# Pose-Group/FAMI-Pose

Measured on AMD Instinct MI355X. Metric: train clips/sec (5-frame 384x288 HRNet-W48), higher is better.
Workload: dtype f32

## Files before the change

fami-pose_amd/csrc/conv.hip:

```cpp
#include "common.h"
#include <type_traits>
#include <string.h>

#include "conv_epi.h"
extern "C" int fami_conv2d_fwd_bnin_ok(int N, int H, int W, int Ci, int Co);
#include "conv_pair.h"
int fami_pair_launch(const PairCapture& c, hipStream_t s);


struct ConvArgs {
  EpiBN e;
  int emode;
  const float* x;
  const float* wp;
  float* y;
  const float* bias;
  const float* addend;
  int N, Hi, Wi, Ci, Ho, Wo, Co;
  int kh, kw, sh, pad, dil;
  int KC, NTt, relu, accumulate, P;
  unsigned x_bytes, wp_bytes;
  int xcd;
  int prio;
  int par;
// ... 2384 lines not shown
      static bool attr2 = false;                                                                                   \
      if (!attr2) {                                                                                                \
        (void)hipFuncSetAttribute((const void*)conv3x3_lds_kernel<T, nt, ksc, 1>, hipFuncAttributeMaxDynamicSharedMemorySize, 156 * 1024); \
        attr2 = true;                                                                                              \
      }                                                                                                            \
      hipLaunchKernelGGL((conv3x3_lds_kernel<T, nt, ksc, 1>), grid, dim3(256), lds, s, a);                         \
    } else                                                                                                         \
    hipLaunchKernelGGL((conv3x3_lds_kernel<T, nt, ksc>), grid, dim3(256), lds, s, a);                              \
    launched = true;                                                                                               \
  }
  FAMI_LDS_CASE(3, 1) FAMI_LDS_CASE(3, 2) FAMI_LDS_CASE(3, 3) FAMI_LDS_CASE(3, 4)
  FAMI_LDS_CASE(4, 1) FAMI_LDS_CASE(4, 2) FAMI_LDS_CASE(4, 3) FAMI_LDS_CASE(4, 4)
#undef FAMI_LDS_CASE
  if (!launched) return 0;
  hipError_t e = hipGetLastError();
  if (e != hipSuccess) {
    fami_set_error(name, hipGetErrorString(e));
    return FAMI_EHIP;
  }
  return 1;
}

static bool wgrad_lin_ok(int H, int W, int Ci, int Co, int kh, int kw, int stride, int pad, int dil) {
  return stride == 1 && 2 * pad == dil * (kh - 1) && 2 * pad == dil * (kw - 1) && kh * kw > 1 && kh * kw <= 9 && W >= 4 &&
         Ci % 16 == 0 && Co % 16 == 0;
}
static bool geom_ok(int kh, int kw, int stride, int pad, int dil) {
  return kh >= 1 && kw >= 1 && kh <= 7 && kw <= 7 && (stride == 1 || stride == 2) && pad >= 0 && dil >= 1;
}
static inline int out_dim(int i, int k, int stride, int pad, int dil) {
  return (i + 2 * pad - dil * (k - 1) - 1) / stride + 1;
}

extern "C" {
int fami_dcn_tune(int mode);
int fami_bn_tune_small(long elems);

int fami_conv_tune(int mt, int nt, int ks) {
  g_force_mt = mt; g_force_nt = nt; g_force_ks = ks;
  return FAMI_OK;
}
void fami_conv_stem_tune(int on);
int fami_conv_tune_lds(int on) {
  if (on == 9000 || on == 9001) {
    fami_conv_stem_tune(on - 9000);
    return FAMI_OK;
  }
  if (on < 0) fami_conv_stem_tune(-1);
  if (on == 10 || on == 11 || on == 20 || on == 21 || on == 30 || on == 31 || (on >= 40 && on <= 42) || (on >= 52 && on <= 54) || (on >= 60 && on <= 62) || on >= 100) {
    fami_conv_t4_tune(on);
    return FAMI_OK;
  }
  g_use_lds = on < 0 ? -1 : (on ? 1 : 0);
  g_lds_sim = on == 2;
  if (on < 0) fami_conv_t4_tune(-1);
  return FAMI_OK;
}
int fami_conv_tune_wgrad_lds(int on) {
  if (on >= 30000) {
    fami_wgrad_s3_tune(on - 30000);
    return FAMI_OK;
  }
  if (on >= 20000) {
    fami_wgrad16_tune(on - 20000);
    return FAMI_OK;
  }
  if (on >= 1000) {
    g_wgrad_ps = on - 1000;
    return FAMI_OK;
  }
  if (on >= 50 && on <= 54) {
    g_wgrad_lin = on - 50;
    return FAMI_OK;
  }
  if (on >= 100) {
    g_wgrad_mt = on - 100;
    return FAMI_OK;
  }
  if (on < 0) {
    fami_wgrad16_tune(-1);
    fami_wgrad_s3_tune(-1);
    g_wgrad_lds = 1;
    g_wgrad_lds_f32 = 2;
    g_wgrad_nsub = 2;
    g_wgrad_lin = 1;
    return FAMI_OK;
  }
  g_wgrad_lds = on ? 1 : 0;
  g_wgrad_lds_f32 = on ? 1 : 0;
  if (on > 1) g_wgrad_nsub = on - 1;
  return FAMI_OK;
}
int fami_conv_tune_xcd(int mode) {
  g_xcd = mode < 0 ? -1 : (mode & 1);
  g_xcd_w = mode < 0 ? 1 : ((mode >> 1) & 1);
  return FAMI_OK;
}
int fami_conv_tune_stages(int stages) {
  if (stages == 120 || stages == 121) {
    g_prio = stages - 120;
    return FAMI_OK;
  }
  if (stages == 110 || stages == 111) {
    g_par = stages - 110;
    return FAMI_OK;
  }
  if (stages == 100 || stages == 101) {
    g_lin_conv = stages - 100;
    return FAMI_OK;
  }
  g_stages = (stages >= 2 && stages <= 4) ? stages : 0;
  return FAMI_OK;
}
int fami_tune_reset(void) {
  fami_conv_tune(0, 0, 0);
  fami_conv_tune_lds(-1);
  fami_conv_tune_wgrad_lds(-1);
  fami_conv_tune_xcd(-1);
  g_stages = 0; g_prio = 0; g_lin_conv = 1; g_par = 1;
  g_wgrad_ps = 0; g_wgrad_mt = 0;
  fami_dcn_tune(-1);
  fami_bn_tune_small(-1);
  return FAMI_OK;
}
int fami_tune_defaults(int f32_split) {
  if (f32_split >= 0) {
    fami_conv_t4_default_split(f32_split);
    fami_wgrad_s3_default(f32_split);
  }
  return fami_tune_reset();
}

long fami_packed_weight_elems(int Co, int Ci, int kh, int kw, int mode) {
  const int kd = mode == 0 ? Ci : Co, nd = mode == 0 ? Co : Ci;
  return pack16_elems(kd, nd, kh * kw) + pack32_elems(kd, nd, kh * kw) + fami_split_image_elems(kd, nd, kh * kw);
}

int fami_pack_conv_weight_f32(const float* w_oihw, float* wp, int Co, int Ci, int kh, int kw, int mode,
                              hipStream_t s) {
  FAMI_REQUIRE(w_oihw && wp && Co > 0 && Ci > 0 && (mode == 0 || mode == 1), "fami_pack_conv_weight_f32", "bad argument");
  const int kd = mode == 0 ? Ci : Co, nd = mode == 0 ? Co : Ci;
  const long total = pack16_elems(kd, nd, kh * kw) + pack32_elems(kd, nd, kh * kw);
  hipLaunchKernelGGL(pack_w_kernel, dim3(fami_ew_grid(total)), dim3(256), 0, s, w_oihw, wp, Co, Ci, kh * kw, mode);
  FAMI_CHECK_LAUNCH("fami_pack_conv_weight_f32");
  if (fami_split_image_elems(kd, nd, kh * kw) > 0) {
    fami_pack_split_single(w_oihw, wp + total, Co, Ci, kh * kw, mode, s);
    FAMI_CHECK_LAUNCH("fami_pack_conv_weight_f32/split");
  }
  return FAMI_OK;
}

static int conv_fwd_f32_impl(const char* nm, const float* x, const float* wp, const float* bias, const float* addend,
                             float* y, int N, int H, int W, int Ci, int Co, int kh, int kw, int stride, int pad, int dil,
                             int relu, int accumulate, const EpiBN& e, hipStream_t s, const XBN& xbn = xbn_none());
int fami_conv2d_fwd_f32(const float* x, const float* wp, const float* bias, const float* addend, float* y, int N,
                        int H, int W, int Ci, int Co, int kh, int kw, int stride, int pad, int dil, int relu,
                        int accumulate, hipStream_t s) {
  return conv_fwd_f32_impl("fami_conv2d_fwd_f32", x, wp, bias, addend, y, N, H, W, Ci, Co, kh, kw, stride, pad, dil, relu,
                           accumulate, epi_none(), s);
}
int fami_conv2d_fwd_stats_f32(const float* x, const float* wp, const float* bias, float* y, int N, int H, int W, int Ci,
                              int Co, int kh, int kw, int stride, int pad, int dil, void* slots, const float* pivot_src,
                              hipStream_t s) {
  FAMI_REQUIRE(slots, "fami_conv2d_fwd_stats_f32", "null slots");
  EpiBN e = epi_none();
// ... 25 lines not shown
                             int relu, int accumulate, const EpiBN& e, hipStream_t s, const XBN& xbn) {
  FAMI_REQUIRE(x && wp && y && N > 0 && H > 0 && W > 0 && Ci > 0 && Co > 0, nm, "bad argument");
  if (!geom_ok(kh, kw, stride, pad, dil)) {
    fami_set_error(nm, "unsupported geometry");
    return FAMI_ESHAPE;
  }
  ConvArgs a;
  a.e = e; a.emode = e.slots ? e.mode : 0;
  a.x = x; a.wp = wp; a.y = y; a.bias = bias; a.addend = addend;
  a.N = N; a.Hi = H; a.Wi = W; a.Ci = Ci;
  a.Ho = out_dim(H, kh, stride, pad, dil); a.Wo = out_dim(W, kw, stride, pad, dil); a.Co = Co;
  a.kh = kh; a.kw = kw; a.sh = stride == 2 ? 1 : 0; a.pad = pad; a.dil = dil;
  a.KC = fami_cdiv(Ci, 16); a.NTt = fami_cdiv(Co, 16); a.relu = relu; a.accumulate = accumulate;
  const long P = (long)N * a.Ho * a.Wo;
  const long xb = (long)N * H * W * Ci * 4, wb = (long)kh * kw * a.KC * a.NTt * 1024;
  FAMI_REQUIRE(P > 0 && P < (1L << 31) && xb < (1L << 31) && wb < (1L << 31), nm, "tensor >= 2 GiB");
  a.P = (int)P; a.x_bytes = (unsigned)xb; a.wp_bytes = (unsigned)wb;
  if (Ci == 3 && !addend && !xbn.on) {
    const int rc = fami_try_conv_stem1(2, x, wp, bias, y, N, H, W, Ci, Co, kh, kw, stride, pad, dil, a.NTt, relu, accumulate, 1, s, nm, e);
    if (rc != 0) return rc < 0 ? rc : FAMI_OK;
  }
  if (kh == 3 && kw == 3 && stride == 1 && pad == 1 && dil == 1 && !addend) {
    const int rc = try_conv3x3_lds<float>(x, wp, bias, y, N, H, W, Ci, Co, a.KC, a.NTt, +1, relu, accumulate, 1, s, nm, e, xbn);
    if (rc != 0) return rc < 0 ? rc : FAMI_OK;
  }
  if (kh == 3 && kw == 3 && stride == 1 && pad == dil && dil > 1 && !addend && !e.slots && !xbn.on && g_use_lds != 0) {
    const int rc = fami_try_conv3x3_t4_dil(2, x, wp, bias, y, N, H, W, Ci, Co, a.KC, a.NTt, +1, relu, accumulate, 1, dil, s, nm);
    if (rc != 0) return rc < 0 ? rc : FAMI_OK;
  }
  if (xbn.on) {
    fami_set_error(nm, "input BatchNorm needs the split-product 3x3 kernel (ask fami_conv2d_xbn_ok_f32 first)");
    return FAMI_ESHAPE;
  }
  return run_igemm(a, 0, s, nm);
}
extern "C" {

static int conv_dgrad_f32_impl(const char* nm, const float* dy, const float* wp, const float* addend, float* dx, int N,
                               int H, int W, int Ci, int Co, int kh, int kw, int stride, int pad, int dil, int accumulate,
                               const EpiBN& e, hipStream_t s);
int fami_conv2d_dgrad_f32(const float* dy, const float* wp, const float* addend, float* dx, int N, int H, int W,
                          int Ci, int Co, int kh, int kw, int stride, int pad, int dil, int accumulate,
                          hipStream_t s) {
  return conv_dgrad_f32_impl("fami_conv2d_dgrad_f32", dy, wp, addend, dx, N, H, W, Ci, Co, kh, kw, stride, pad, dil,
                             accumulate, epi_none(), s);
}
int fami_conv2d_dgrad_bnstats_f32(const float* dy, const float* wp, float* dx, int N, int H, int W, int Ci, int Co,
                                  int kh, int kw, int stride, int pad, int dil, int accumulate, const float* z,
                                  const float* yrelu, const float* mean, const float* invstd, const float* gamma,
                                  const float* beta, int relu, void* slots, hipStream_t s) {
  FAMI_REQUIRE(slots && z && mean && invstd && gamma && beta && (relu != 1 || yrelu) && relu >= 0 && relu <= 2,
               "fami_conv2d_dgrad_bnstats_f32", "bad argument");
  EpiBN e = epi_none();
  e.slots = reinterpret_cast<double*>(slots); e.ns = bn_slots(Ci); e.mode = 2; e.relu = relu; e.C = Ci;
  e.z = z; e.yr = yrelu; e.mean = mean; e.invstd = invstd; e.gamma = gamma; e.beta = beta;
  return conv_dgrad_f32_impl("fami_conv2d_dgrad_bnstats_f32", dy, wp, nullptr, dx, N, H, W, Ci, Co, kh, kw, stride, pad,
                             dil, accumulate, e, s);
}
}
static int conv_dgrad_f32_impl(const char* nm, const float* dy, const float* wp, const float* addend, float* dx, int N,
                               int H, int W, int Ci, int Co, int kh, int kw, int stride, int pad, int dil, int accumulate,
                               const EpiBN& e, hipStream_t s) {
  FAMI_REQUIRE(dy && wp && dx && N > 0 && H > 0 && W > 0 && Ci > 0 && Co > 0, nm, "bad argument");
  if (!geom_ok(kh, kw, stride, pad, dil)) {
    fami_set_error(nm, "unsupported geometry");
    return FAMI_ESHAPE;
  }
  ConvArgs a;
  a.e = e; a.emode = e.slots ? e.mode : 0;
  a.x = dy; a.wp = wp; a.y = dx; a.bias = nullptr; a.addend = addend;
  a.N = N; a.Hi = out_dim(H, kh, stride, pad, dil); a.Wi = out_dim(W, kw, stride, pad, dil); a.Ci = Co;
  a.Ho = H; a.Wo = W; a.Co = Ci;
  a.kh = kh; a.kw = kw; a.sh = stride == 2 ? 1 : 0; a.pad = pad; a.dil = dil;
  a.KC = fami_cdiv(Co, 16); a.NTt = fami_cdiv(Ci, 16); a.relu = 0; a.accumulate = accumulate;
  const long P = (long)N * H * W;
  const long xb = (long)N * a.Hi * a.Wi * Co * 4, wb = (long)kh * kw * a.KC * a.NTt * 1024;
  FAMI_REQUIRE(P > 0 && P < (1L << 31) && xb < (1L << 31) && wb < (1L << 31), nm, "tensor >= 2 GiB");
  a.P = (int)P; a.x_bytes = (unsigned)xb; a.wp_bytes = (unsigned)wb;
  if (kh == 3 && kw == 3 && stride == 1 && pad == 1 && dil == 1 && !addend) {
    const int rc = try_conv3x3_lds<float>(dy, wp, nullptr, dx, N, H, W, Co, Ci, a.KC, a.NTt, -1, 0, accumulate, 1, s, nm, e);
    if (rc != 0) return rc < 0 ? rc : FAMI_OK;
  }
  if (kh == 3 && kw == 3 && stride == 1 && pad == dil && dil > 1 && !addend && !e.slots && g_use_lds != 0) {
    const int rc = fami_try_conv3x3_t4_dil(2, dy, wp, nullptr, dx, N, H, W, Co, Ci, a.KC, a.NTt, -1, 0, accumulate, 1, dil, s, nm);
    if (rc != 0) return rc < 0 ? rc : FAMI_OK;
  }
  return run_igemm(a, 1, s, nm);
}
extern "C" {

struct WgradPlan { int MT, NT, ciBlocks, coBlocks, psplit, chunk, pertap, w8; long P; };
static bool wgrad_lin_ok(int H, int W, int Ci, int Co, int kh, int kw, int stride, int pad, int dil);
static WgradPlan wgrad_plan(int N, int H, int W, int Ci, int Co, int kh, int kw, int stride, int pad, int dil, int w8 = 0) {
  WgradPlan q;
  const int Ho = out_dim(H, kh, stride, pad, dil), Wo = out_dim(W, kw, stride, pad, dil);
  q.P = (long)N * Ho * Wo;
  q.MT = pick_small(fami_cdiv(Ci, 16));
  q.NT = pick_small(fami_cdiv(Co, 16));
  if (g_wgrad_mt > 0 && g_wgrad_mt <= q.MT) q.MT = g_wgrad_mt;
  q.ciBlocks = fami_cdiv(fami_cdiv(Ci, 16), q.MT);
  q.coBlocks = fami_cdiv(fami_cdiv(Co, 16), q.NT);
  q.pertap = (kh * kw > 1 && kh * kw <= 9) ? 1 : 0;
  const long by = q.pertap ? (long)q.ciBlocks * q.coBlocks : (long)kh * kw * q.ciBlocks * q.coBlocks;
  long ps = ((q.pertap ? (g_wgrad_ps ? g_wgrad_ps : 512) : 1024) + by - 1) / by;
  q.w8 = 0;
  if (w8 == 3) w8 = 256 / by >= 16 ? 2 : 1;
  if (w8 && q.pertap && kh * kw == 9 && ps >= 9) {
    q.w8 = w8;
    const long T = (g_wgrad_ps ? g_wgrad_ps : (w8 == 2 ? 256 : 512)) / by;
    ps = T * 8 / 9;
    while (ps > 1 && ps + (ps + 7) / 8 > T) --ps;
    if (ps < 1) ps = 1;
    if (w8 == 2) ps *= 2;
  }
  const long maxps = q.pertap ? (q.P + 63) / 64 : (q.P + 255) / 256;
  if (ps > maxps) ps = maxps;
  if (ps < 1) ps = 1;
// ... 62 lines not shown
  G = (P + chunk - 1) / chunk;
  q.G = (int)G;
  q.chunk = (int)chunk;
  q.xbytes = (int)((chunk + 2 * (W + 1)) * q.xrow);
  q.lds = ((size_t)q.xbytes + (size_t)chunk * q.yrow + 16) * 4;
  q.ok = P < (1L << 31) && G < 65536;
  return q;
}

int fami_conv2d_xbn_ok(int N, int H, int W, int Ci, int Co) {
  return (g_use_lds != 0 && g_wgrad_lds && fami_conv_t4_eligible16(N, H, W, Ci, Co) &&
          fami_wgrad16_slabs(N, H, W, Ci, Co, 3, 1, 1, 1) > 0) ? 1 : 0;
}
long fami_conv2d_wgrad_workspace(int N, int H, int W, int Ci, int Co, int kh, int kw, int stride, int pad, int dil) {
  if (!geom_ok(kh, kw, stride, pad, dil)) return -1;
  const WgradPlan q = wgrad_plan(N, H, W, Ci, Co, kh, kw, stride, pad, dil);
  long need = (long)q.psplit * Co * Ci * kh * kw * (long)sizeof(float);
  const WgradLdsPlan l = wgrad_lds_plan(N, H, W, Ci, Co, kh, kw, stride, pad, dil);
  if (l.ok) {
    const long nl = (long)l.G * Co * Ci * 9 * (long)sizeof(float);
    if (nl > need) need = nl;
  }
  const WgradLdsPlan f = wgrad_lds_plan_f32(N, H, W, Ci, Co, kh, kw, stride, pad, dil);
  if (f.ok) {
    const long nl = (long)f.G * Co * Ci * 9 * (long)sizeof(float);
    if (nl > need) need = nl;
  }
  if (kh == kw) {
    const long nl = fami_wgrad16_slabs(N, H, W, Ci, Co, kh, stride, pad, dil) * Co * Ci * kh * kw * (long)sizeof(float);
    if (nl > need) need = nl;
  }
  if (kh == 3 && kw == 3 && stride == 1 && pad == 1 && dil == 1) {
    const long nl = fami_wgrad_s3_slabs(N, H, W, Ci, Co) * Co * Ci * 9 * (long)sizeof(float);
    if (nl > need) need = nl;
  }
  return need;
}

}

template <typename T>
static int wgrad_impl(const T* x, const T* dy, float* dw, float* workspace, long ws_bytes, int N, int H, int W, int Ci,
                      int Co, int kh, int kw, int stride, int pad, int dil, int accumulate, hipStream_t s,
                      const char* nm) {
  FAMI_REQUIRE(x && dy && dw && workspace && N > 0 && H > 0 && W > 0 && Ci > 0 && Co > 0, nm, "bad argument");
  if (!geom_ok(kh, kw, stride, pad, dil)) {
    fami_set_error(nm, "unsupported geometry");
    return FAMI_ESHAPE;
  }
  const bool lin = std::is_same<T, float>::value && g_wgrad_lin && wgrad_lin_ok(H, W, Ci, Co, kh, kw, stride, pad, dil);
  const WgradPlan q = wgrad_plan(N, H, W, Ci, Co, kh, kw, stride, pad, dil, !lin ? 0 : (g_wgrad_lin == 1 ? 3 : (g_wgrad_lin == 3 ? 1 : (g_wgrad_lin == 4 ? 2 : 0))));
  const long need = (long)q.psplit * Co * Ci * kh * kw * (long)sizeof(float);
  FAMI_REQUIRE(ws_bytes >= need, nm, "workspace too small");
  FAMI_REQUIRE(q.P < (1L << 31), nm, "size out of range");
  WgradArgs<T> a;
  a.x = x; a.dy = dy; a.part = workspace;
  a.N = N; a.H = H; a.W = W; a.Ci = Ci;
  a.Ho = out_dim(H, kh, stride, pad, dil); a.Wo = out_dim(W, kw, stride, pad, dil); a.Co = Co;
  a.kh = kh; a.kw = kw; a.sh = stride == 2 ? 1 : 0; a.pad = pad; a.dil = dil;
  a.P = (int)q.P; a.chunk = q.chunk; a.ciBlocks = q.ciBlocks; a.coBlocks = q.coBlocks; a.xcd = g_xcd_w; a.prio = g_prio;
  const long xb = (long)N * H * W * Ci * (long)sizeof(T), yb = q.P * Co * (long)sizeof(T);
  FAMI_REQUIRE(xb < (1L << 31) && yb < (1L << 31), nm, "tensor >= 2 GiB");
  a.x_bytes = (unsigned)xb; a.dy_bytes = (unsigned)yb;
  if (q.pertap) {
    const dim3 grid(q.w8 ? q.psplit + (q.psplit + 7) / 8 : q.psplit, q.ciBlocks * q.coBlocks), block(q.w8 ? 512 * q.w8 : kh * kw * 64);
    const size_t lin_lds = q.w8 == 2 ? (size_t)8 * q.MT * q.NT * 1024 : 0;
// ... 111 lines not shown
  if (rc != 0) {
    fami_set_error(name, "no kernel instance for tile shape");
    return FAMI_ESHAPE;
  }
  FAMI_CHECK_LAUNCH(name);
  return FAMI_OK;
}

extern "C" {

static int wgrad_f32_entry(const float* x, const float* dy, float* dw, float* workspace, long ws_bytes, int N, int H,
                           int W, int Ci, int Co, int kh, int kw, int stride, int pad, int dil, int accumulate,
                           hipStream_t s, const XBN& xbn);
int fami_conv2d_wgrad_f32(const float* x, const float* dy, float* dw, float* workspace, long ws_bytes, int N, int H,
                          int W, int Ci, int Co, int kh, int kw, int stride, int pad, int dil, int accumulate,
                          hipStream_t s) {
  return wgrad_f32_entry(x, dy, dw, workspace, ws_bytes, N, H, W, Ci, Co, kh, kw, stride, pad, dil, accumulate, s, xbn_none());
}
static int wgrad_f32_entry(const float* x, const float* dy, float* dw, float* workspace, long ws_bytes, int N, int H,
                           int W, int Ci, int Co, int kh, int kw, int stride, int pad, int dil, int accumulate,
                           hipStream_t s, const XBN& xbn) {
  if (kh == 3 && kw == 3 && stride == 1 && pad == 1 && dil == 1 && x && dy && dw && workspace) {
    const int G = fami_try_wgrad_s3(x, dy, workspace, ws_bytes, N, H, W, Ci, Co, s, "fami_conv2d_wgrad_f32", xbn);
    if (G < 0) return G;
    if (G > 0) {
      launch_reduce_taps(workspace, dw, Co, Ci, 9, G, accumulate, s);
      FAMI_CHECK_LAUNCH("fami_conv2d_wgrad_f32/reduce");
      return FAMI_OK;
    }
  }
  if (xbn.on) {
    fami_set_error("fami_conv2d_wgrad_defer_xbn_f32", "input BatchNorm needs the split-product kernel (ask fami_conv2d_xbn_ok_f32 first)");
    return FAMI_ESHAPE;
  }
  WgradLdsPlan l = g_wgrad_lds_f32 ? wgrad_lds_plan_f32(N, H, W, Ci, Co, kh, kw, stride, pad, dil) : WgradLdsPlan{0};
  if (g_wgrad_lds_f32 == 2 && l.ok &&
      (l.ciBlocks * l.coBlocks < 64 || (g_wgrad_lin && wgrad_lin_ok(H, W, Ci, Co, kh, kw, stride, pad, dil))))
    l.ok = 0;
  if (l.ok && x && dy && dw && workspace && ((reinterpret_cast<uintptr_t>(x) | reinterpret_cast<uintptr_t>(dy)) & 15) == 0) {
    const long need = (long)l.G * Co * Ci * 9 * (long)sizeof(float);
    FAMI_REQUIRE(ws_bytes >= need, "fami_conv2d_wgrad_f32", "workspace too small");
    WgradLdsArgsF a;
    a.x = x; a.dy = dy; a.part = workspace;
    a.N = N; a.H = H; a.W = W; a.Ci = Ci; a.Co = Co; a.P = N * H * W;
    a.chunk = l.chunk; a.ciBlocks = l.ciBlocks; a.coBlocks = l.coBlocks; a.xcd = g_xcd_w;
    a.CiB = 16 * l.CIT; a.CoB = 16 * l.COT; a.xrow = l.xrow; a.yrow = l.yrow; a.xfloats = l.xbytes;
    const dim3 grid(l.G, l.ciBlocks * l.coBlocks);
    bool ok = false;
#define FAMI_WF_CASE(cit, cot)                                                                                        \
  if (l.CIT == cit && l.COT == cot) {                                                                                 \
    static bool attr = false;                                                                                         \
    if (!attr) {                                                                                                      \
      (void)hipFuncSetAttribute((const void*)conv_wgrad_lds_f32_kernel<cit, cot>, hipFuncAttributeMaxDynamicSharedMemorySize, 160 * 1024); \
      attr = true;                                                                                                    \
    }                                                                                                                 \
    hipLaunchKernelGGL((conv_wgrad_lds_f32_kernel<cit, cot>), grid, dim3(512), l.lds, s, a);                          \
    ok = true;                                                                                                        \
  }
    FAMI_WF_CASE(1, 1) FAMI_WF_CASE(1, 2) FAMI_WF_CASE(1, 3) FAMI_WF_CASE(1, 4) FAMI_WF_CASE(2, 1) FAMI_WF_CASE(2, 2)
    FAMI_WF_CASE(2, 3) FAMI_WF_CASE(2, 4) FAMI_WF_CASE(3, 1) FAMI_WF_CASE(3, 2) FAMI_WF_CASE(3, 3) FAMI_WF_CASE(3, 4)
    FAMI_WF_CASE(4, 1) FAMI_WF_CASE(4, 2) FAMI_WF_CASE(4, 3) FAMI_WF_CASE(4, 4)
#undef FAMI_WF_CASE
    if (ok) {
      FAMI_CHECK_LAUNCH("fami_conv2d_wgrad_f32/lds");
      launch_reduce_taps(workspace, dw, Co, Ci, 9, l.G, accumulate, s);
      FAMI_CHECK_LAUNCH("fami_conv2d_wgrad_f32/reduce");
// ... 437 lines not shown
```

fami-pose_amd/csrc/conv_epi.h:

```cpp
#pragma once
#include "common.h"

struct EpiBN {
  double* slots;
  int ns, mode, relu, C;
  const float* pivot_src;
  const void* z;
  const void* yr;
  const float *mean, *invstd, *gamma, *beta;
};
static inline EpiBN epi_none() {
  EpiBN e;
  e.slots = nullptr; e.ns = 1; e.mode = 0; e.relu = 0; e.C = 0; e.pivot_src = nullptr; e.z = nullptr; e.yr = nullptr;
  e.mean = e.invstd = e.gamma = e.beta = nullptr;
  return e;
}
#if defined(__HIP_DEVICE_COMPILE__)
typedef const __attribute__((address_space(4))) EpiBN* EpiPtr;
__device__ __forceinline__ EpiPtr epi_late(unsigned off) {
  const __attribute__((address_space(4))) char* k =
      (const __attribute__((address_space(4))) char*)__builtin_amdgcn_kernarg_segment_ptr() + off;
  asm volatile("" : "+s"(k) : : "memory");
  return (EpiPtr)k;
}
// ... 61 lines not shown
}
template <typename H>
__device__ __forceinline__ u32x4 xbn_piece(u32x4 raw, const float* sc, const float* sf) {
  typedef H hx8 __attribute__((ext_vector_type(8)));
  typedef float f32x8 __attribute__((ext_vector_type(8)));
  f32x8 v = __builtin_convertvector(__builtin_bit_cast(hx8, raw), f32x8);
#pragma unroll
  for (int j = 0; j < 8; ++j) v[j] = fmaxf(__builtin_fmaf(v[j], sc[j], sf[j]), 0.f);
  return __builtin_bit_cast(u32x4, __builtin_convertvector(v, hx8));
}

int fami_try_conv3x3_t4(int half_kind, const void* x, const void* wp, const float* bias, void* y, int N, int H, int W, int Ci,
                        int Co, int KC, int NTt, int sgn, int relu, int accumulate, int out_f32, hipStream_t s,
                        const char* name, const EpiBN& epi, const XBN& xbn = xbn_none());
int fami_try_conv3x3_t4_dil(int half_kind, const void* x, const void* wp, const float* bias, void* y, int N, int H, int W, int Ci,
                            int Co, int KC, int NTt, int sgn, int relu, int accumulate, int out_f32, int dil, hipStream_t s,
                            const char* name);
void fami_conv_t4_tune(int on);
void fami_conv_t4_default_split(int on);
int fami_conv_t4_eligible16(int N, int H, int W, int Ci, int Co);
int fami_conv_t4_eligible_s3(int N, int H, int W, int Ci, int Co);

long fami_wgrad16_slabs(int N, int H, int W, int Ci, int Co, int k, int st, int pad, int dil);
int fami_try_wgrad16(int half_kind, const void* x, const void* dy, float* part, long ws_bytes, int N, int H, int W, int Ci,
                     int Co, int k, int st, int pad, int dil, hipStream_t s, const char* name, const XBN& xbn = xbn_none());
void fami_wgrad16_tune(int on);

long fami_wgrad_s3_slabs(int N, int H, int W, int Ci, int Co);
int fami_try_wgrad_s3(const float* x, const float* dy, float* part, long ws_bytes, int N, int H, int W, int Ci, int Co,
                      hipStream_t s, const char* name, const XBN& xbn = xbn_none());
void fami_wgrad_s3_tune(int on);
void fami_wgrad_s3_default(int on);

long fami_split_image_elems(int kd, int nd, int taps);
void fami_pack_split_single(const float* w_oihw, float* split, int Co, int Ci, int taps, int mode, hipStream_t s);
void fami_pack_split_batch(const float* params, float* packed, const void* desc, int n, hipStream_t s);
int fami_try_conv3x3_t5(int half_kind, const void* x, const void* wp, const float* bias, void* y, int N, int H, int W, int Ci,
                        int Co, int KC, int NTt, int sgn, int relu, int accumulate, int out_f32, hipStream_t s,
                        const char* name, const EpiBN& epi, const XBN& xbn);
void fami_conv_t5_tune(int on);
int fami_conv_t5_eligible_s3(int N, int H, int W, int Ci, int Co);

int fami_try_conv3x3_t6(int half_kind, const void* x, const void* wp, const float* bias, void* y, int N, int H, int W, int Ci,
                        int Co, int KC, int NTt, int sgn, int relu, int accumulate, int out_f32, hipStream_t s,
                        const char* name, const EpiBN& epi, const XBN& xbn);
extern "C" int fami_conv_t6_eligible(int N, int H, int W, int Ci, int Co);
void fami_conv_t6_tune(int on);
```

fami-pose_amd/csrc/route.h:

```cpp
#pragma once
#include "../../include/fami_route.h"
extern "C" fami_route_t* fami_rt(void);

#define g_dcn_gather (fami_rt()->dcn_gather)
#define g_dcn_abl (fami_rt()->dcn_abl)
#define g_dcn_win_r (fami_rt()->dcn_win_r)
#define g_dcn_ksplit (fami_rt()->dcn_ksplit)
#define g_dcn_pf (fami_rt()->dcn_pf)
#define g_dcn_bwd2 (fami_rt()->dcn_bwd2)
#define g_dcn_bwd2_cap (fami_rt()->dcn_bwd2_cap)
#define g_dcn_bwd2_stage (fami_rt()->dcn_bwd2_stage)
#define g_dcn_bwd_abl (fami_rt()->dcn_bwd_abl)
#define g_dcn_bwd_scatter (fami_rt()->dcn_bwd_scatter)
#define g_prio (fami_rt()->prio)
#define g_lin_conv (fami_rt()->lin_conv)
#define g_par (fami_rt()->par)
#define g_force_mt (fami_rt()->force_mt)
#define g_force_nt (fami_rt()->force_nt)
#define g_force_ks (fami_rt()->force_ks)
#define g_stages (fami_rt()->stages)
#define g_use32 (fami_rt()->use32)
#define g_xcd_w (fami_rt()->xcd_w)
#define g_xcd (fami_rt()->xcd)
#define g_use_lds (fami_rt()->use_lds)
// ... 26 lines not shown
#define g_t5_min_tiles (fami_rt()->t5_min_tiles)
#define g_use_t6 (fami_rt()->use_t6)
#define g_t6_rows (fami_rt()->t6_rows)
#define g_t6_min_jobs (fami_rt()->t6_min_jobs)
#define g_t6_mt (fami_rt()->t6_mt)
#define g_t7_target (fami_rt()->t7_target)
#define g_use_t7 (fami_rt()->use_t7)
#define g_t7_rows (fami_rt()->t7_rows)
#define g_t7_c64 (fami_rt()->t7_c64)
#define g_bn_in (fami_rt()->bn_in)
#define g_bwd_pair (fami_rt()->bwd_pair)
#define g_pair_wg6_target (fami_rt()->pair_wg6_target)
#define g_wg6_s2 (fami_rt()->wg6_s2)
#define g_wg6_dil (fami_rt()->wg6_dil)
#define g_wg6_c42 (fami_rt()->wg6_c42)
#define g_wg6_c4 (fami_rt()->wg6_c4)
#define g_wg6 (fami_rt()->wg6)
#define g_wg6_nu (fami_rt()->wg6_nu)
#define g_wg6_target (fami_rt()->wg6_target)
#define g_wg6_target_c4 (fami_rt()->wg6_target_c4)
#define g_wg1 (fami_rt()->wg1)
#define g_wg1_target (fami_rt()->wg1_target)
#define g_wgs (fami_rt()->wgs)
#define g_wg16_abl (fami_rt()->wg16_abl)
#define g_wg16 (fami_rt()->wg16)
#define g_wg16_bt (fami_rt()->wg16_bt)
#define g_wg16_target (fami_rt()->wg16_target)
#define g_wg16_general (fami_rt()->wg16_general)
#define g_wg16_bt18 (fami_rt()->wg16_bt18)
#define g_wgs3 (fami_rt()->wgs3)
#define g_wgs3_bt (fami_rt()->wgs3_bt)
#define g_wgs3_target (fami_rt()->wgs3_target)
#define g_wgs3_default (fami_rt()->wgs3_default)
#define g_bn_small_elems (fami_rt()->bn_small_elems)
#define g_bn2_maxg (fami_rt()->bn2_maxg)

static inline void fami_route_set_defaults(fami_route_t* q) {
  q->size = (int)sizeof(fami_route_t);
  q->dcn_gather = -1;
  q->dcn_abl = 0;
  q->dcn_win_r = 0;
  q->dcn_ksplit = 1;
  q->dcn_pf = 0;
  q->dcn_bwd2 = 1;
  q->dcn_bwd2_cap = 36;
  q->dcn_bwd2_stage = 1;
  q->dcn_bwd_abl = 0;
  q->dcn_bwd_scatter = -1;
  q->prio = 0;
  q->lin_conv = 1;
  q->par = 1;
  q->force_mt = 0;
  q->force_nt = 0;
  q->force_ks = 0;
  q->stages = 0;
  q->use32 = 1;
  q->xcd_w = 1;
  q->xcd = -1;
  q->use_lds = -1;
  q->lds_sim = 0;
  q->wgrad_nsub = 2;
  q->wgrad_ps = 0;
  q->wgrad_mt = 0;
  q->wgrad_lds = 1;
  q->wgrad_lds_f32 = 2;
  q->wgrad_lin = 1;
// ... 19 lines not shown
  q->t5_min_tiles = 0;
  q->use_t6 = 1;
  q->t6_rows = 0;
  q->t6_min_jobs = 96;
  q->t6_mt = 0;
  q->t7_target = 240;
  q->use_t7 = 1;
  q->t7_rows = 0;
  q->t7_c64 = 1;
  q->bn_in = 1;
  q->bwd_pair = 1;
  q->pair_wg6_target = 64;
  q->wg6_s2 = 1;
  q->wg6_dil = 1;
  q->wg6_c42 = 1;
  q->wg6_c4 = 1;
  q->wg6 = 1;
  q->wg6_nu = 0;
  q->wg6_target = 80;
  q->wg6_target_c4 = 160;
  q->wg1 = 1;
  q->wg1_target = 192;
  q->wgs = 1;
  q->wg16_abl = 0;
  q->wg16 = 1;
  q->wg16_bt = 0;
  q->wg16_target = 0;
  q->wg16_general = 1;
  q->wg16_bt18 = 0;
  q->wgs3 = 1;
  q->wgs3_bt = 0;
  q->wgs3_target = 0;
  q->wgs3_default = 1;
  q->bn_small_elems = 32768;
  q->bn2_maxg = 512;
}
```

include/fami.h:

```cpp
#ifndef FAMI_H
#define FAMI_H
#ifdef __cplusplus
extern "C" {
#endif

typedef void* fami_stream_t;

#include "fami_route.h"
long fami_route_size(void);
int fami_route_init(fami_route_t* route);
int fami_route_bind(fami_route_t* route);

const char* fami_version(void);
const char* fami_last_error(void);
int fami_device_info(int device, int* info, char* name, int name_len);

int fami_conv_tune(int mt, int nt, int ks);
int fami_conv_tune_lds(int on);
int fami_conv_tune_wgrad_lds(int on);
int fami_conv_tune_xcd(int mode);
int fami_conv_tune_stages(int stages);
int fami_tune_reset(void);
int fami_tune_defaults(int f32_split);
int fami_conv_t5_eligible(int N, int H, int W, int Ci, int Co);
int fami_conv_t6_eligible(int N, int H, int W, int Ci, int Co);
long fami_packed_weight_elems(int Co, int Ci, int kh, int kw, int mode);
int fami_pack_conv_weight_f32(const float* w_oihw, float* wp, int Co, int Ci, int kh, int kw, int mode,
                              fami_stream_t stream);
int fami_pack_conv_weights_batch_f32(const float* params, float* packed, const void* desc, int n, fami_stream_t stream);
int fami_conv2d_fwd_f32(const float* x, const float* wp, const float* bias, const float* addend, float* y, int N,
                        int H, int W, int Ci, int Co, int kh, int kw, int stride, int pad, int dil, int relu,
                        int accumulate, fami_stream_t stream);
int fami_conv2d_dgrad_f32(const float* dy, const float* wp, const float* addend, float* dx, int N, int H, int W,
                          int Ci, int Co, int kh, int kw, int stride, int pad, int dil, int accumulate,
                          fami_stream_t stream);
int fami_conv2d_fwd_stats_f32(const float* x, const float* wp, const float* bias, float* y, int N, int H, int W, int Ci,
                              int Co, int kh, int kw, int stride, int pad, int dil, void* slots, const float* pivot_src,
                              fami_stream_t stream);
int fami_conv2d_dgrad_bnstats_f32(const float* dy, const float* wp, float* dx, int N, int H, int W, int Ci, int Co,
                                  int kh, int kw, int stride, int pad, int dil, int accumulate, const float* z,
                                  const float* yrelu, const float* mean, const float* invstd, const float* gamma,
                                  const float* beta, int relu, void* slots, fami_stream_t stream);
long fami_conv2d_wgrad_workspace(int N, int H, int W, int Ci, int Co, int kh, int kw, int stride, int pad, int dil);
int fami_wgrad_reduce_desc_longs(void);
int fami_wgrad_reduce_batch(const long* descs, int n, fami_stream_t stream);
int fami_conv2d_wgrad_defer_f32(const float* x, const float* dy, float* dw, float* workspace, long ws_bytes, int N,
                                int H, int W, int Ci, int Co, int kh, int kw, int stride, int pad, int dil,
                                int accumulate, long* desc_out, fami_stream_t stream);
int fami_conv2d_wgrad_f32(const float* x, const float* dy, float* dw, float* workspace, long ws_bytes, int N, int H,
                          int W, int Ci, int Co, int kh, int kw, int stride, int pad, int dil, int accumulate,
                          fami_stream_t stream);

long fami_bn_workspace(int C);
int fami_bn_stats_f32(const float* x, long P, int C, float* mean, float* invstd, float* running_mean,
                      float* running_var, float momentum, float eps, float* ws, fami_stream_t stream);
int fami_bn_train_fwd_f32(const float* x, const float* residual, float* y, const float* gamma, const float* beta,
                          float* mean, float* invstd, float* running_mean, float* running_var, long P, int C,
                          int relu, float momentum, float eps, float* ws, fami_stream_t stream);
// ... 446 lines not shown
```

include/fami_route.h:

```cpp
#ifndef FAMI_ROUTE_H
#define FAMI_ROUTE_H
#ifdef __cplusplus
extern "C" {
#endif

typedef struct fami_route_t {
  int size;
  int  dcn_gather;
  int  dcn_abl;
  int  dcn_win_r;
  int  dcn_ksplit;
  int  dcn_pf;
  int  dcn_bwd2;
  int  dcn_bwd2_cap;
  int  dcn_bwd2_stage;
  int  dcn_bwd_abl;
  int  dcn_bwd_scatter;
  int  prio;
  int  lin_conv;
  int  par;
  int  force_mt;
  int  force_nt;
  int  force_ks;
  int  stages;
// ... 30 lines not shown
  int  t5_min_tiles;
  int  use_t6;
  int  t6_rows;
  int  t6_min_jobs;
  int  t6_mt;
  int  t7_target;
  int  use_t7;
  int  t7_rows;
  int  t7_c64;
  int  bn_in;
  int  bwd_pair;
  int  pair_wg6_target;
  int  wg6_s2;
  int  wg6_dil;
  int  wg6_c42;
  int  wg6_c4;
  int  wg6;
  int  wg6_nu;
  int  wg6_target;
  int  wg6_target_c4;
  int  wg1;
  int  wg1_target;
  int  wgs;
  int  wg16_abl;
  int  wg16;
  int  wg16_bt;
  int  wg16_target;
  int  wg16_general;
  int  wg16_bt18;
  int  wgs3;
  int  wgs3_bt;
  int  wgs3_target;
  int  wgs3_default;
  long bn_small_elems;
  int  bn2_maxg;
} fami_route_t;

#ifdef __cplusplus
}
#endif
#endif
```

Measured before the change: 90.98.

## Add streaming MFMA kernels for large 1x1 conv dgrad and wgrad

Adds a dedicated 1x1 convolution path: a persistent GEMM kernel with double-buffered LDS pixel tiles and MFMA 32x32x2 f32 for forward/dgrad (with optional BN-stats epilogue), and a wgrad kernel that streams pixel chunks into per-workgroup slabs reduced afterwards. By default it routes only large-P wgrad and Ci=64 dgrad shapes to the new kernels, replacing the generic implicit-GEMM path. This targets the generic path's overhead on skinny 1x1 GEMMs, at the cost of extra workspace for the slabs and more tuning knobs.

```diff
diff --git a/fami-pose_amd/csrc/conv.hip b/fami-pose_amd/csrc/conv.hip
--- a/fami-pose_amd/csrc/conv.hip
+++ b/fami-pose_amd/csrc/conv.hip
@@ -2440,6 +2440,11 @@
   return (i + 2 * pad - dil * (k - 1) - 1) / stride + 1;
 }
 
+static inline unsigned long c1s_addr_or(const void* a, const void* b, const void* c, const void* d, const void* e) {
+  return (unsigned long)(reinterpret_cast<uintptr_t>(a) | reinterpret_cast<uintptr_t>(b) | reinterpret_cast<uintptr_t>(c) |
+                         reinterpret_cast<uintptr_t>(d) | reinterpret_cast<uintptr_t>(e));
+}
+
 extern "C" {
 int fami_dcn_tune(int mode);
 int fami_bn_tune_small(long elems);
@@ -2505,6 +2510,14 @@
   return FAMI_OK;
 }
 int fami_conv_tune_stages(int stages) {
+  if (stages >= 130 && stages <= 132) {
+    g_c1s = stages - 130;
+    return FAMI_OK;
+  }
+  if (stages >= 1000) {
+    g_c1s_maxwg = stages - 1000;
+    return FAMI_OK;
+  }
   if (stages == 120 || stages == 121) {
     g_prio = stages - 120;
     return FAMI_OK;
@@ -2527,6 +2540,7 @@
   fami_conv_tune_xcd(-1);
   g_stages = 0; g_prio = 0; g_lin_conv = 1; g_par = 1;
   g_wgrad_ps = 0; g_wgrad_mt = 0;
+  g_c1s = 2; g_c1s_maxwg = 0;
   fami_dcn_tune(-1);
   fami_bn_tune_small(-1);
   return FAMI_OK;
@@ -2539,6 +2553,11 @@
   return fami_tune_reset();
 }
 
+int fami_conv1x1_stream_eligible(int N, int H, int W, int Ci, int Co, int kh, int kw, int stride, int pad, int dil, int what,
+                                 long addr_or) {
+  if (N <= 0 || H <= 0 || W <= 0 || Ci <= 0 || Co <= 0) return 0;
+  return fami_c1s_route((long)N * H * W, Ci, Co, kh, kw, stride, pad, dil, what, (unsigned long)addr_or);
+}
 long fami_packed_weight_elems(int Co, int Ci, int kh, int kw, int mode) {
   const int kd = mode == 0 ? Ci : Co, nd = mode == 0 ? Co : Ci;
   return pack16_elems(kd, nd, kh * kw) + pack32_elems(kd, nd, kh * kw) + fami_split_image_elems(kd, nd, kh * kw);
@@ -2630,6 +2649,11 @@
     fami_set_error(nm, "input BatchNorm needs the split-product 3x3 kernel (ask fami_conv2d_xbn_ok_f32 first)");
     return FAMI_ESHAPE;
   }
+  if (kh == 1 && kw == 1 && !addend && !relu && (!e.slots || e.mode == 1) &&
+      fami_c1s_route(P, Ci, Co, kh, kw, stride, pad, dil, 0, c1s_addr_or(x, y, wp, bias, e.slots ? e.pivot_src : nullptr))) {
+    const int rc = fami_try_conv1x1s(x, wp + pack16_elems(Ci, Co, 1), bias, y, P, Ci, Co, accumulate, e, s, nm);
+    if (rc != 0) return rc < 0 ? rc : FAMI_OK;
+  }
   return run_igemm(a, 0, s, nm);
 }
 extern "C" {
@@ -2681,6 +2705,11 @@
   }
   if (kh == 3 && kw == 3 && stride == 1 && pad == dil && dil > 1 && !addend && !e.slots && g_use_lds != 0) {
     const int rc = fami_try_conv3x3_t4_dil(2, dy, wp, nullptr, dx, N, H, W, Co, Ci, a.KC, a.NTt, -1, 0, accumulate, 1, dil, s, nm);
+    if (rc != 0) return rc < 0 ? rc : FAMI_OK;
+  }
+  if (kh == 1 && kw == 1 && !addend && !e.slots &&
+      fami_c1s_route(P, Ci, Co, kh, kw, stride, pad, dil, 1, c1s_addr_or(dy, dx, wp, nullptr, nullptr))) {
+    const int rc = fami_try_conv1x1s(dy, wp + pack16_elems(Co, Ci, 1), nullptr, dx, P, Co, Ci, accumulate, e, s, nm);
     if (rc != 0) return rc < 0 ? rc : FAMI_OK;
   }
   return run_igemm(a, 1, s, nm);
@@ -2809,6 +2838,10 @@
   }
   if (kh == 3 && kw == 3 && stride == 1 && pad == 1 && dil == 1) {
     const long nl = fami_wgrad_s3_slabs(N, H, W, Ci, Co) * Co * Ci * 9 * (long)sizeof(float);
+    if (nl > need) need = nl;
+  }
+  if (fami_c1s_route((long)N * H * W, Ci, Co, kh, kw, stride, pad, dil, 2, 0)) {
+    const long nl = fami_wgrad1x1s_slabs((long)N * H * W, Ci, Co) * Co * Ci * (long)sizeof(float);
     if (nl > need) need = nl;
   }
   return need;
@@ -2986,6 +3019,16 @@
   if (xbn.on) {
     fami_set_error("fami_conv2d_wgrad_defer_xbn_f32", "input BatchNorm needs the split-product kernel (ask fami_conv2d_xbn_ok_f32 first)");
     return FAMI_ESHAPE;
+  }
+  if (x && dy && dw && workspace && N > 0 && H > 0 && W > 0 && Ci > 0 && Co > 0 &&
+      fami_c1s_route((long)N * H * W, Ci, Co, kh, kw, stride, pad, dil, 2, c1s_addr_or(x, dy, workspace, nullptr, nullptr))) {
+    const int G = fami_try_wgrad1x1s(x, dy, workspace, ws_bytes, (long)N * H * W, Ci, Co, s, "fami_conv2d_wgrad_f32");
+    if (G < 0) return G;
+    if (G > 0) {
+      launch_reduce_taps(workspace, dw, Co, Ci, 1, G, accumulate, s);
+      FAMI_CHECK_LAUNCH("fami_conv2d_wgrad_f32/reduce");
+      return FAMI_OK;
+    }
   }
   WgradLdsPlan l = g_wgrad_lds_f32 ? wgrad_lds_plan_f32(N, H, W, Ci, Co, kh, kw, stride, pad, dil) : WgradLdsPlan{0};
   if (g_wgrad_lds_f32 == 2 && l.ok &&
diff --git a/fami-pose_amd/csrc/conv_1x1s.hip b/fami-pose_amd/csrc/conv_1x1s.hip
--- /dev/null
+++ b/fami-pose_amd/csrc/conv_1x1s.hip
@@ -0,0 +1,379 @@
+#include "common.h"
+#include "conv_epi.h"
+
+typedef float f32x16 __attribute__((ext_vector_type(16)));
+#define C1S_OOB 0x80000000u
+
+constexpr int C1S_PX = 64;
+constexpr int C1S_ROW = 68;
+constexpr int C1S_BUF = C1S_PX * C1S_ROW;
+constexpr int C1S_SCR = 32 * 33;
+constexpr long C1S_MIN_P = 100000;
+
+struct C1sArgs {
+  EpiBN e;
+  int emode;
+  const float* x;
+  const float* wp;
+  float* y;
+  const float* bias;
+  int P, K, Nn, accumulate, ntiles;
+  unsigned x_bytes, wp_bytes;
+};
+
+template <int NTW>
+__global__ __launch_bounds__(256, 3) void conv1x1s_kernel(C1sArgs p) {
+  extern __shared__ __attribute__((aligned(16))) float sm[];
+  const int tid = threadIdx.x, lane = tid & 63;
+  const int wave = __builtin_amdgcn_readfirstlane(tid >> 6);
+  const int col = lane & 31, h = lane >> 5;
+  const int pg = wave & 1, cg = wave >> 1;
+  const int nk = p.K >> 6, NTt = p.Nn >> 5;
+  const int emode = p.emode;
+  int tile = blockIdx.x;
+  if (tile >= p.ntiles) return;
+  const __amdgpu_buffer_rsrc_t rx = __builtin_amdgcn_make_buffer_rsrc((void*)p.x, 0, (int)p.x_bytes, 0x00020000);
+  const __amdgpu_buffer_rsrc_t rw = __builtin_amdgcn_make_buffer_rsrc((void*)p.wp, 0, (int)p.wp_bytes, 0x00020000);
+
+  const int spx = tid >> 4, spc = (tid & 15) * 4;
+  f32x4 st[4];
+  auto fetch = [&](int t, int kch) {
+#pragma unroll
+    for (int j = 0; j < 4; ++j) {
+      const int m = t * C1S_PX + j * 16 + spx;
+      const unsigned off = m < p.P ? ((unsigned)m * (unsigned)p.K + (unsigned)(kch * 64 + spc)) * 4u : C1S_OOB;
+      st[j] = __builtin_bit_cast(f32x4, __builtin_amdgcn_raw_buffer_load_b128(rx, off, 0, 0));
+    }
+  };
+  auto stash = [&](int buf) {
+#pragma unroll
+    for (int j = 0; j < 4; ++j) *reinterpret_cast<f32x4*>(sm + buf * C1S_BUF + (j * 16 + spx) * C1S_ROW + spc) = st[j];
+  };
+
+  constexpr bool SPLIT = NTW <= 2;
+  f32x16 acc[NTW], part[SPLIT ? NTW : 1];
+  float es[NTW], eq[NTW];
+#pragma unroll
+  for (int nt = 0; nt < NTW; ++nt) es[nt] = eq[nt] = 0.f;
+
+  fetch(tile, 0);
+  stash(0);
+  __syncthreads();
+  int buf = 0;
+  for (;;) {
+#pragma unroll
+    for (int nt = 0; nt < NTW; ++nt)
+#pragma unroll
+      for (int r = 0; r < 16; ++r) acc[nt][r] = 0.f;
+    for (int kch = 0; kch < nk; ++kch) {
+      int ntile = tile, nkch = kch + 1;
+      if (nkch == nk) {
+        nkch = 0;
+        ntile = tile + gridDim.x;
+      }
+      const bool more = ntile < p.ntiles;
+      if (more) fetch(ntile, nkch);
+      {
+        const float* xs = sm + buf * C1S_BUF + (pg * 32 + col) * C1S_ROW + h * 4;
+        const unsigned wb = (unsigned)((kch * 8) * NTt + cg * NTW) * 1024u + (unsigned)lane * 16u;
+        const unsigned wstep = (unsigned)NTt * 1024u;
+        f32x4 a0, a1, b0[NTW], b1[NTW];
+        auto load = [&](int ks, f32x4& a, f32x4(&b)[NTW]) {
+          a = *reinterpret_cast<const f32x4*>(xs + ks * 8);
+#pragma unroll
+          for (int nt = 0; nt < NTW; ++nt)
+            b[nt] = __builtin_bit_cast(f32x4, __builtin_amdgcn_raw_buffer_load_b128(rw, wb + ks * wstep + nt * 1024u, 0, 0));
+        };
+        auto mma = [&](const f32x4& a, const f32x4(&b)[NTW]) {
+#pragma unroll
+          for (int t = 0; t < 4; ++t)
+#pragma unroll
+            for (int nt = 0; nt < NTW; ++nt) {
+              if constexpr (SPLIT) part[nt] = __builtin_amdgcn_mfma_f32_32x32x2f32(b[nt][t], a[t], part[nt], 0, 0, 0);
+              else acc[nt] = __builtin_amdgcn_mfma_f32_32x32x2f32(b[nt][t], a[t], acc[nt], 0, 0, 0);
+            }
+        };
+        if constexpr (SPLIT) {
+#pragma unroll
+          for (int nt = 0; nt < NTW; ++nt)
+#pragma unroll
+            for (int r = 0; r < 16; ++r) part[nt][r] = 0.f;
+        }
+        load(0, a0, b0);
+#pragma unroll
+        for (int ks = 0; ks < 8; ks += 2) {
+          load(ks + 1, a1, b1);
+          mma(a0, b0);
+          if (ks + 2 < 8) load(ks + 2, a0, b0);
+          mma(a1, b1);
+        }
+        if constexpr (SPLIT) {
+#pragma unroll
+          for (int nt = 0; nt < NTW; ++nt) acc[nt] += part[nt];
+        }
+      }
+      if (more) stash(buf ^ 1);
+      if (kch == nk - 1) {
+        const int m = tile * C1S_PX + pg * 32 + col;
+        const bool pv = m < p.P;
+        EpiPtr e = epi_late(__builtin_offsetof(C1sArgs, e));
+        float* sc = sm + 2 * C1S_BUF + wave * C1S_SCR;
+#pragma unroll
+        for (int nt = 0; nt < NTW; ++nt) {
+#pragma unroll
+          for (int q = 0; q < 4; ++q) {
+            const int co0 = (cg * NTW + nt) * 32 + 8 * q + 4 * h;
+            f32x4 v = {acc[nt][4 * q], acc[nt][4 * q + 1], acc[nt][4 * q + 2], acc[nt][4 * q + 3]};
+            if (p.bias) v += *reinterpret_cast<const f32x4*>(p.bias + co0);
+            if (pv) {
+              float* dst = p.y + (long)m * p.Nn + co0;
+              if (p.accumulate) v += *reinterpret_cast<const f32x4*>(dst);
+              *reinterpret_cast<f32x4*>(dst) = v;
+            }
+            if (emode == 1) {
+              f32x4 ek = {0.f, 0.f, 0.f, 0.f};
+              if (e->pivot_src) ek = *reinterpret_cast<const f32x4*>(e->pivot_src + co0);
+#pragma unroll
+              for (int r = 0; r < 4; ++r) sc[(8 * q + 4 * h + r) * 33 + col] = pv ? v[r] - ek[r] : 0.f;
+            }
+          }
+          if (emode == 1) {
+            __builtin_amdgcn_wave_barrier();
+            asm volatile("" ::: "memory");
+            float s1 = 0.f, s2 = 0.f;
+#pragma unroll
+            for (int j = 0; j < 16; ++j) {
+              const float d = sc[col * 33 + h * 16 + j];
+              s1 += d;
+              s2 = __builtin_fmaf(d, d, s2);
+            }
+            es[nt] += s1;
+            eq[nt] += s2;
+            __builtin_amdgcn_wave_barrier();
+            asm volatile("" ::: "memory");
+          }
+        }
+      }
+      __syncthreads();
+      buf ^= 1;
+    }
+    tile += gridDim.x;
+    if (tile >= p.ntiles) break;
+  }
+  if (emode == 1) {
+    EpiPtr e = epi_late(__builtin_offsetof(C1sArgs, e));
+    const int eC = e->C;
+    double* srow = e->slots + (long)(blockIdx.x % e->ns) * 2 * eC;
+#pragma unroll
+    for (int nt = 0; nt < NTW; ++nt) {
+      es[nt] += __shfl_xor(es[nt], 32, 64);
+      eq[nt] += __shfl_xor(eq[nt], 32, 64);
+      if (pg == 1 && h == 0) {
+        sm[((cg * NTW + nt) * 2 + 0) * 32 + col] = es[nt];
+        sm[((cg * NTW + nt) * 2 + 1) * 32 + col] = eq[nt];
+      }
+    }
+    __syncthreads();
+    if (pg == 0 && h == 0) {
+#pragma unroll
+      for (int nt = 0; nt < NTW; ++nt) {
+        const int co = (cg * NTW + nt) * 32 + col;
+        unsafeAtomicAdd(srow + co, (double)(es[nt] + sm[((cg * NTW + nt) * 2 + 0) * 32 + col]));
+        unsafeAtomicAdd(srow + eC + co, (double)(eq[nt] + sm[((cg * NTW + nt) * 2 + 1) * 32 + col]));
+      }
+    }
+    if (blockIdx.x == 0)
+      for (int c = tid; c < p.Nn; c += 256) bn_slots_pivot(e->slots, eC)[c] = e->pivot_src ? e->pivot_src[c] : 0.f;
+  }
+}
+
+struct W1sArgs {
+  const float* x;
+  const float* dy;
+  float* part;
+  int P, NU, per;
+  unsigned x_bytes, dy_bytes;
+};
+
+template <int CIT, int COT>
+__global__ __launch_bounds__(256) void wgrad1x1s_kernel(W1sArgs p) {
+  constexpr int WGO = COT % 4 == 0 ? 4 : 2, WGI = 4 / WGO, WCI = CIT / WGI, WCO = COT / WGO;
+  constexpr int Ci = CIT * 32, Co = COT * 32, BUF = 32 * (Ci + Co);
+  static_assert(CIT % WGI == 0 && WCI * WCO <= 4, "tile block");
+  extern __shared__ __attribute__((aligned(16))) float sm[];
+  const int tid = threadIdx.x, lane = tid & 63;
+  const int wave = __builtin_amdgcn_readfirstlane(tid >> 6);
+  const int col = lane & 31, h = lane >> 5;
+  const int wi = wave % WGI, wo = wave / WGI;
+  const int g = blockIdx.x;
+  const int u0 = g * p.per, u1 = min(p.NU, u0 + p.per);
+  const __amdgpu_buffer_rsrc_t rx = __builtin_amdgcn_make_buffer_rsrc((void*)p.x, 0, (int)p.x_bytes, 0x00020000);
+  const __amdgpu_buffer_rsrc_t ry = __builtin_amdgcn_make_buffer_rsrc((void*)p.dy, 0, (int)p.dy_bytes, 0x00020000);
+
+  f32x4 sx[2][CIT], sy[2][COT];
+  auto fetch = [&](int u, f32x4(&vx)[CIT], f32x4(&vy)[COT]) {
+#pragma unroll
+    for (int j = 0; j < CIT; ++j) {
+      const int q = j * 256 + tid;
+      const int m = u * 32 + q / (Ci / 4);
+      const unsigned off = m < p.P ? ((unsigned)u * (32u * Ci) + (unsigned)q * 4u) * 4u : C1S_OOB;
+      vx[j] = __builtin_bit_cast(f32x4, __builtin_amdgcn_raw_buffer_load_b128(rx, off, 0, 0));
+    }
+#pragma unroll
+    for (int j = 0; j < COT; ++j) {
+      const int q = j * 256 + tid;
+      const int m = u * 32 + q / (Co / 4);
+      const unsigned off = m < p.P ? ((unsigned)u * (32u * Co) + (unsigned)q * 4u) * 4u : C1S_OOB;
+      vy[j] = __builtin_bit_cast(f32x4, __builtin_amdgcn_raw_buffer_load_b128(ry, off, 0, 0));
+    }
+  };
+  auto stash = [&](int buf, const f32x4(&vx)[CIT], const f32x4(&vy)[COT]) {
+#pragma unroll
+    for (int j = 0; j < CIT; ++j) *reinterpret_cast<f32x4*>(sm + buf * BUF + (j * 256 + tid) * 4) = vx[j];
+#pragma unroll
+    for (int j = 0; j < COT; ++j) *reinterpret_cast<f32x4*>(sm + buf * BUF + 32 * Ci + (j * 256 + tid) * 4) = vy[j];
+  };
+
+  f32x16 acc[WCI][WCO];
+#pragma unroll
+  for (int a = 0; a < WCI; ++a)
+#pragma unroll
+    for (int b = 0; b < WCO; ++b)
+#pragma unroll
+      for (int r = 0; r < 16; ++r) acc[a][b][r] = 0.f;
+  auto compute = [&](int buf) {
+    const float* xs = sm + buf * BUF + h * Ci + (wi * WCI) * 32 + col;
+    const float* ys = sm + buf * BUF + 32 * Ci + h * Co + (wo * WCO) * 32 + col;
+#pragma unroll
+    for (int s = 0; s < 16; ++s) {
+      float av[WCI], bv[WCO];
+#pragma unroll
+      for (int a = 0; a < WCI; ++a) av[a] = xs[(2 * s) * Ci + a * 32];
+#pragma unroll
+      for (int b = 0; b < WCO; ++b) bv[b] = ys[(2 * s) * Co + b * 32];
+#pragma unroll
+      for (int a = 0; a < WCI; ++a)
+#pragma unroll
+        for (int b = 0; b < WCO; ++b) acc[a][b] = __builtin_amdgcn_mfma_f32_32x32x2f32(av[a], bv[b], acc[a][b], 0, 0, 0);
+    }
+  };
+
+  const int n = u1 - u0;
+  if (n > 0) {
+    fetch(u0, sx[0], sy[0]);
+    stash(0, sx[0], sy[0]);
+    if (n > 1) fetch(u0 + 1, sx[1], sy[1]);
+  }
+  __syncthreads();
+  for (int r = 0; r < n; r += 2) {
+    if (r + 2 < n) fetch(u0 + r + 2, sx[0], sy[0]);
+    compute(0);
+    if (r + 1 < n) stash(1, sx[1], sy[1]);
+    __syncthreads();
+    if (r + 1 >= n) break;
+    if (r + 3 < n) fetch(u0 + r + 3, sx[1], sy[1]);
+    compute(1);
+    if (r + 2 < n) stash(0, sx[0], sy[0]);
+    __syncthreads();
+  }
+  float* slab = p.part + (long)g * (Ci * Co);
+#pragma unroll
+  for (int a = 0; a < WCI; ++a)
+#pragma unroll
+    for (int b = 0; b < WCO; ++b)
+#pragma unroll
+      for (int r = 0; r < 16; ++r) {
+        const int ci = (wi * WCI + a) * 32 + (r & 3) + 8 * (r >> 2) + 4 * h;
+        slab[ci * Co + (wo * WCO + b) * 32 + col] = acc[a][b][r];
+      }
+}
+
+static bool c1s_shape_ok(long P, int Ci, int Co) {
+  return P > 0 && Ci % 64 == 0 && Co % 64 == 0 && Ci <= 256 && Co <= 256 && Ci * Co <= 16384 &&
+         P * (Ci > Co ? Ci : Co) * 4 < (1L << 31);
+}
+int fami_c1s_route(long P, int Ci, int Co, int kh, int kw, int stride, int pad, int dil, int what, unsigned long addr_or) {
+  if (!g_c1s || kh != 1 || kw != 1 || stride != 1 || pad != 0 || dil != 1 || (addr_or & 15) != 0) return 0;
+  if (what < 0 || what > 2 || !c1s_shape_ok(P, Ci, Co)) return 0;
+  return (g_c1s == 1 || (P >= C1S_MIN_P && (what == 2 || (what == 1 && Ci == 64)))) ? 1 : 0;
+}
+
+int fami_try_conv1x1s(const float* x, const float* wp32, const float* bias, float* y, long P, int K, int Nn, int accumulate,
+                      const EpiBN& e, hipStream_t s, const char* name) {
+  if (!c1s_shape_ok(P, K, Nn) || (e.slots && e.mode != 1)) return 0;
+  C1sArgs a;
+  a.e = e; a.emode = e.slots ? 1 : 0;
+  a.x = x; a.wp = wp32; a.y = y; a.bias = bias;
+  a.P = (int)P; a.K = K; a.Nn = Nn; a.accumulate = accumulate;
+  a.ntiles = fami_cdiv(P, C1S_PX);
+  a.x_bytes = (unsigned)(P * K * 4); a.wp_bytes = (unsigned)((long)K * Nn * 4);
+  int G = g_c1s_maxwg > 0 ? g_c1s_maxwg : 768;
+  if (G > a.ntiles) G = a.ntiles;
+  const size_t lds = (size_t)(2 * C1S_BUF + (a.emode ? 4 * C1S_SCR : 0)) * sizeof(float);
+  switch (Nn / 64) {
+    case 1: hipLaunchKernelGGL((conv1x1s_kernel<1>), dim3(G), dim3(256), lds, s, a); break;
+    case 2: hipLaunchKernelGGL((conv1x1s_kernel<2>), dim3(G), dim3(256), lds, s, a); break;
+    case 3: hipLaunchKernelGGL((conv1x1s_kernel<3>), dim3(G), dim3(256), lds, s, a); break;
+    default: hipLaunchKernelGGL((conv1x1s_kernel<4>), dim3(G), dim3(256), lds, s, a); break;
+  }
+  hipError_t err = hipGetLastError();
+  if (err != hipSuccess) {
+    fami_set_error(name, hipGetErrorString(err));
+    return FAMI_EHIP;
+  }
+  return 1;
+}
+
+struct W1sPlan { int ok, NU, per, G; };
+static W1sPlan w1s_plan(long P, int Ci, int Co) {
+  W1sPlan q;
+  q.ok = c1s_shape_ok(P, Ci, Co) ? 1 : 0;
+  q.NU = q.per = q.G = 0;
+  if (!q.ok) return q;
+  q.NU = fami_cdiv(P, 32);
+  int G = g_c1s_maxwg > 0 ? g_c1s_maxwg : 256;
+  if (G > q.NU) G = q.NU;
+  q.per = fami_cdiv(q.NU, G);
+  q.G = fami_cdiv(q.NU, q.per);
+  return q;
+}
+long fami_wgrad1x1s_slabs(long P, int Ci, int Co) {
+  const W1sPlan q = w1s_plan(P, Ci, Co);
+  return q.ok ? q.G : 0;
+}
+
+int fami_try_wgrad1x1s(const float* x, const float* dy, float* part, long ws_bytes, long P, int Ci, int Co, hipStream_t s,
+                       const char* name) {
+  const W1sPlan q = w1s_plan(P, Ci, Co);
+  if (!q.ok) return 0;
+  if (ws_bytes < (long)q.G * Ci * Co * (long)sizeof(float)) {
+    fami_set_error(name, "workspace too small");
+    return FAMI_EARG;
+  }
+  W1sArgs a;
+  a.x = x; a.dy = dy; a.part = part;
+  a.P = (int)P; a.NU = q.NU; a.per = q.per;
+  a.x_bytes = (unsigned)(P * Ci * 4); a.dy_bytes = (unsigned)(P * Co * 4);
+  const size_t lds = (size_t)2 * 32 * (Ci + Co) * sizeof(float);
+  bool ok = false;
+#define FAMI_W1S_CASE(cit, cot)                                                                                          \
+  if (!ok && Ci == cit * 32 && Co == cot * 32) {                                                                         \
+    static bool attr = false;                                                                                            \
+    if (!attr) {                                                                                                         \
+      (void)hipFuncSetAttribute((const void*)wgrad1x1s_kernel<cit, cot>, hipFuncAttributeMaxDynamicSharedMemorySize, 80 * 1024); \
+      attr = true;                                                                                                       \
+    }                                                                                                                    \
+    hipLaunchKernelGGL((wgrad1x1s_kernel<cit, cot>), dim3(q.G), dim3(256), lds, s, a);                                   \
+    ok = true;                                                                                                           \
+  }
+  FAMI_W1S_CASE(2, 2) FAMI_W1S_CASE(2, 4) FAMI_W1S_CASE(2, 6) FAMI_W1S_CASE(2, 8)
+  FAMI_W1S_CASE(4, 2) FAMI_W1S_CASE(4, 4) FAMI_W1S_CASE(6, 2) FAMI_W1S_CASE(8, 2)
+#undef FAMI_W1S_CASE
+  if (!ok) return 0;
+  hipError_t err = hipGetLastError();
+  if (err != hipSuccess) {
+    fami_set_error(name, hipGetErrorString(err));
+    return FAMI_EHIP;
+  }
+  return q.G;
+}
diff --git a/fami-pose_amd/csrc/conv_epi.h b/fami-pose_amd/csrc/conv_epi.h
--- a/fami-pose_amd/csrc/conv_epi.h
+++ b/fami-pose_amd/csrc/conv_epi.h
@@ -117,6 +117,13 @@
 void fami_wgrad_s3_tune(int on);
 void fami_wgrad_s3_default(int on);
 
+int fami_c1s_route(long P, int Ci, int Co, int kh, int kw, int stride, int pad, int dil, int what, unsigned long addr_or);
+int fami_try_conv1x1s(const float* x, const float* wp32, const float* bias, float* y, long P, int K, int Nn, int accumulate,
+                      const EpiBN& e, hipStream_t s, const char* name);
+long fami_wgrad1x1s_slabs(long P, int Ci, int Co);
+int fami_try_wgrad1x1s(const float* x, const float* dy, float* part, long ws_bytes, long P, int Ci, int Co, hipStream_t s,
+                       const char* name);
+
 long fami_split_image_elems(int kd, int nd, int taps);
 void fami_pack_split_single(const float* w_oihw, float* split, int Co, int Ci, int taps, int mode, hipStream_t s);
 void fami_pack_split_batch(const float* params, float* packed, const void* desc, int n, hipStream_t s);
diff --git a/fami-pose_amd/csrc/route.h b/fami-pose_amd/csrc/route.h
--- a/fami-pose_amd/csrc/route.h
+++ b/fami-pose_amd/csrc/route.h
@@ -82,6 +82,8 @@
 #define g_wgs3_bt (fami_rt()->wgs3_bt)
 #define g_wgs3_target (fami_rt()->wgs3_target)
 #define g_wgs3_default (fami_rt()->wgs3_default)
+#define g_c1s (fami_rt()->c1s)
+#define g_c1s_maxwg (fami_rt()->c1s_maxwg)
 #define g_bn_small_elems (fami_rt()->bn_small_elems)
 #define g_bn2_maxg (fami_rt()->bn2_maxg)
 
@@ -167,6 +169,8 @@
   q->wgs3_bt = 0;
   q->wgs3_target = 0;
   q->wgs3_default = 1;
+  q->c1s = 2;
+  q->c1s_maxwg = 0;
   q->bn_small_elems = 32768;
   q->bn2_maxg = 512;
 }
diff --git a/include/fami.h b/include/fami.h
--- a/include/fami.h
+++ b/include/fami.h
@@ -24,6 +24,8 @@
 int fami_tune_defaults(int f32_split);
 int fami_conv_t5_eligible(int N, int H, int W, int Ci, int Co);
 int fami_conv_t6_eligible(int N, int H, int W, int Ci, int Co);
+int fami_conv1x1_stream_eligible(int N, int H, int W, int Ci, int Co, int kh, int kw, int stride, int pad, int dil, int what,
+                                 long addr_or);
 long fami_packed_weight_elems(int Co, int Ci, int kh, int kw, int mode);
 int fami_pack_conv_weight_f32(const float* w_oihw, float* wp, int Co, int Ci, int kh, int kw, int mode,
                               fami_stream_t stream);
diff --git a/include/fami_route.h b/include/fami_route.h
--- a/include/fami_route.h
+++ b/include/fami_route.h
@@ -86,6 +86,8 @@
   int  wgs3_bt;
   int  wgs3_target;
   int  wgs3_default;
+  int  c1s;
+  int  c1s_maxwg;
   long bn_small_elems;
   int  bn2_maxg;
 } fami_route_t;
```

Result: no change. 91.54, median of 5 (+0.6%).
